# yigolden/JpegLibrary

Hardware: AMD Instinct MI355X
Metric: Mpixels/s decoded, 4K 4:2:0 baseline Q75 RST=4, 1 & 8 GPU vs CPU ref (higher is better)
Workload: dtype f32; 1 GPU; 1024 x 3840x2160 420 baseline Q75 DRI=4 per GPU, output interleaved_u8 resident in HBM; images_per_gpu=1024

## Files before the change

### jpeglibrary_amd/csrc/k3_idct.hip

```cpp
#include <hip/hip_runtime.h>
#include <stdint.h>

#include <algorithm>
#include <atomic>
#include <cstdio>
#include <cstdlib>

#include "common.h"
#include "kernels.h"
#include "encode_kernels.h"
#include "kernels_device.h"
#include "k3_index_math.h"

namespace jpgpu {


__device__ constexpr uint8_t kNat[64] = {0,  1,  8,  16, 9,  2,  3,  10, 17, 24, 32, 25, 18, 11, 4,  5,  12, 19, 26, 33, 40, 48,
                                         41, 34, 27, 20, 13, 6,  7,  14, 21, 28, 35, 42, 49, 56, 57, 50, 43, 36, 29, 22, 15, 23,
                                         30, 37, 44, 51, 58, 59, 52, 45, 38, 31, 39, 46, 53, 60, 61, 54, 47, 55, 62, 63};

static_assert(kIdctBlocksPerWg == 256, "the split form's reciprocals are exact for tiles of up to 256 blocks");
static_assert(kMaxBlocksPerMcu == 16, "kRecip16 and the 16-bit reciprocals of the split form cover 1..16 blocks per MCU");
__device__ constexpr uint32_t kRecip16[kMaxBlocksPerMcu + 1] = {0, 65536, 32768, 21846, 16384, 13108, 10923, 9363, 8192, 7282, 6554, 5958, 5462, 5042, 4682, 4370, 4096};

#define JPGPU_IDCT8(y0, y1, y2, y3, y4, y5, y6, y7)                     \
    {                                                                   \
        float mz0 = y1 + y7;                                            \
        float mz2 = y3 + y7;                                            \
        float mz1 = y3 + y5;                                            \
        float mz3 = y1 + y5;                                            \
        float mz4 = (mz0 + mz1) * 1.175875602f;                         \
        mz2 = (mz2 * -1.961570560f) + mz4;                              \
        mz3 = (mz3 * -0.390180644f) + mz4;                              \
        mz0 = mz0 * -0.899976223f;                                      \
        mz1 = mz1 * -2.562915447f;                                      \
        const float mb3 = ((y7 * 0.298631336f) + mz0) + mz2;            \
        const float mb2 = ((y5 * 2.053119869f) + mz1) + mz3;            \
        const float mb1 = ((y3 * 3.072711026f) + mz1) + mz2;            \
        const float mb0 = ((y1 * 1.501321110f) + mz0) + mz3;            \
        mz4 = (y2 + y6) * 0.541196100f;                                 \
        mz0 = y0 + y4;                                                  \
        mz1 = y0 - y4;                                                  \
        mz2 = mz4 + (y6 * -1.847759065f);                               \
        mz3 = mz4 + (y2 * 0.765366865f);                                \
        const float a0 = mz0 + mz3;                                     \
        const float a3 = mz0 - mz3;                                     \
        const float a1 = mz1 + mz2;                                     \
        const float a2 = mz1 - mz2;                                     \
        y0 = a0 + mb0;                                                  \
        y7 = a0 - mb0;                                                  \
        y1 = a1 + mb1;                                                  \
        y6 = a1 - mb1;                                                  \
        y2 = a2 + mb2;                                                  \
        y5 = a2 - mb2;                                                  \
        y3 = a3 + mb3;                                                  \
        y4 = a3 - mb3;                                                  \
    }

__device__ __forceinline__ void block_dequant(const uint8_t *c_lds, uint32_t swz, const uint16_t *q_lds, float (&f)[64]) {
#pragma unroll
    for (int piece = 0; piece < 8; piece++) {
        const uint4 cv = *reinterpret_cast<const uint4 *>(c_lds + ((piece ^ swz) * 16));
        const uint4 qv = reinterpret_cast<const uint4 *>(q_lds)[piece];
        const uint32_t cw[4] = {cv.x, cv.y, cv.z, cv.w};
        const uint32_t qw[4] = {qv.x, qv.y, qv.z, qv.w};
#pragma unroll
        for (int j = 0; j < 8; j++) {
            const int k = piece * 8 + j;
            const uint32_t w = cw[j >> 1], q = qw[j >> 1];
            const int32_t c = (j & 1) ? ((int32_t)w >> 16) : (int32_t)(int16_t)(w & 0xFFFF);
            const int32_t qq = (j & 1) ? (int32_t)(q >> 16) : (int32_t)(q & 0xFFFF);
            f[kNat[k]] = (float)(qq * c);
        }
    }
}

typedef float float2v __attribute__((ext_vector_type(2)));
typedef short short2v __attribute__((ext_vector_type(2)));
typedef unsigned short ushort2v __attribute__((ext_vector_type(2)));

template <typename T>
__device__ __forceinline__ void idct8(T &y0, T &y1, T &y2, T &y3, T &y4, T &y5, T &y6, T &y7) {
    T mz0 = y1 + y7;
    T mz2 = y3 + y7;
    T mz1 = y3 + y5;
    T mz3 = y1 + y5;
    T mz4 = (mz0 + mz1) * 1.175875602f;
    mz2 = (mz2 * -1.961570560f) + mz4;
    mz3 = (mz3 * -0.390180644f) + mz4;
    mz0 = mz0 * -0.899976223f;
    mz1 = mz1 * -2.562915447f;
    const T mb3 = ((y7 * 0.298631336f) + mz0) + mz2;
    const T mb2 = ((y5 * 2.053119869f) + mz1) + mz3;
    const T mb1 = ((y3 * 3.072711026f) + mz1) + mz2;
    const T mb0 = ((y1 * 1.501321110f) + mz0) + mz3;
    mz4 = (y2 + y6) * 0.541196100f;
    mz0 = y0 + y4;
    mz1 = y0 - y4;
    mz2 = mz4 + (y6 * -1.847759065f);
    mz3 = mz4 + (y2 * 0.765366865f);
    const T a0 = mz0 + mz3;
    const T a3 = mz0 - mz3;
    const T a1 = mz1 + mz2;
    const T a2 = mz1 - mz2;
    y0 = a0 + mb0;
    y7 = a0 - mb0;
    y1 = a1 + mb1;
    y6 = a1 - mb1;
    y2 = a2 + mb2;
    y5 = a2 - mb2;
    y3 = a3 + mb3;
    y4 = a3 - mb3;
}

__device__ __forceinline__ void block_idct(const float (&f)[64], int32_t level_shift, uint32_t (&out)[32]) {
#if defined(JPGPU_K3_PRICE)
#pragma unroll
    for (int i = 0; i < 32; i++) out[i] = (__builtin_bit_cast(uint32_t, f[2 * i]) >> 16) | (__builtin_bit_cast(uint32_t, f[2 * i + 1]) & 0xFFFF0000u) | (uint32_t)level_shift;
    return;
#endif
    float2v a[4][8];
#pragma unroll
    for (int r2 = 0; r2 < 4; r2++)
#pragma unroll
        for (int c = 0; c < 8; c++) a[r2][c] = float2v{f[(2 * r2) * 8 + c], f[(2 * r2 + 1) * 8 + c]};
#pragma unroll
    for (int r2 = 0; r2 < 4; r2++) idct8(a[r2][0], a[r2][1], a[r2][2], a[r2][3], a[r2][4], a[r2][5], a[r2][6], a[r2][7]);
    float2v b[8][4];
#pragma unroll
    for (int r2 = 0; r2 < 4; r2++)
#pragma unroll
        for (int c2 = 0; c2 < 4; c2++) {
            b[2 * r2][c2] = float2v{a[r2][2 * c2].x, a[r2][2 * c2 + 1].x};
            b[2 * r2 + 1][c2] = float2v{a[r2][2 * c2].y, a[r2][2 * c2 + 1].y};
        }
#pragma unroll
    for (int c2 = 0; c2 < 4; c2++) idct8(b[0][c2], b[1][c2], b[2][c2], b[3][c2], b[4][c2], b[5][c2], b[6][c2], b[7][c2]);
    const uint32_t shift2 = ((uint32_t)level_shift & 0xFFFFu) * 0x00010001u;
#pragma unroll
    for (int r = 0; r < 8; r++)
#pragma unroll
        for (int c2 = 0; c2 < 4; c2++) {
            const float2v v = b[r][c2] * 0.1250f;
            const int32_t x = (int32_t)__builtin_rintf(v.x);
            const int32_t y = (int32_t)__builtin_rintf(v.y);
            const uint32_t pk = ((uint32_t)x & 0xFFFFu) | ((uint32_t)y << 16);
            const short2v sum = __builtin_bit_cast(short2v, pk) + __builtin_bit_cast(short2v, shift2);
            out[r * 4 + c2] = __builtin_bit_cast(uint32_t, sum);
        }
}

__device__ __forceinline__ uint32_t clamp2_u8(uint32_t pk) {
    short2v v = __builtin_bit_cast(short2v, pk);
    v = __builtin_elementwise_max(v, short2v{0, 0});
    v = __builtin_elementwise_min(v, short2v{255, 255});
    return __builtin_bit_cast(uint32_t, v);
}
__device__ __forceinline__ uint32_t pack4_u8(uint32_t pk01, uint32_t pk23) {
    return __builtin_amdgcn_perm(clamp2_u8(pk23), clamp2_u8(pk01), 0x06040200u);
}
struct ScaleTo8 {
    uint32_t shift2, max2, mul2, rem2, mask2;
    bool expand;
};
__device__ __forceinline__ ScaleTo8 scale_to_8(uint32_t precision) {
    const uint32_t p = precision < 1u ? 1u : (precision > 16u ? 16u : precision);
    ScaleTo8 k;
    k.expand = p < 8u;
    const uint32_t pe = k.expand ? p : 1u;
    const uint32_t m = (uint32_t)(0x010101110955FFull >> (8u * (pe - 1u))) & 0xFFu;
    const uint32_t rem = 8u % pe;
    k.shift2 = (k.expand ? 0u : p - 8u) * 0x00010001u;
    k.max2 = ((1u << pe) - 1u) * 0x00010001u;
    k.mul2 = m * 0x00010001u;
    k.rem2 = rem * 0x00010001u;
    k.mask2 = ((1u << rem) - 1u) * 0x00010001u;
    return k;
}
__device__ __forceinline__ uint32_t shift_sat2_u8(uint32_t pk, const ScaleTo8 &k) {
    const uint32_t t = __builtin_bit_cast(uint32_t, __builtin_bit_cast(short2v, pk) >> __builtin_bit_cast(short2v, k.shift2));
    uint32_t r;
    asm("v_sat_pk_u8_i16 %0, %1" : "=v"(r) : "v"(t));
    return r;
}
__device__ __forceinline__ uint32_t expand2_u8(uint32_t pk, const ScaleTo8 &k) {
    short2v v = __builtin_bit_cast(short2v, pk);
    v = __builtin_elementwise_max(v, short2v{0, 0});
    v = __builtin_elementwise_min(v, __builtin_bit_cast(short2v, k.max2));
    const ushort2v r = __builtin_bit_cast(ushort2v, v) * __builtin_bit_cast(ushort2v, k.mul2);
    const ushort2v hi = r << __builtin_bit_cast(ushort2v, k.rem2);
    return __builtin_bit_cast(uint32_t, hi) | (__builtin_bit_cast(uint32_t, r) & k.mask2);
}
__device__ __forceinline__ uint32_t pick4(uint32_t lo, uint32_t hi, uint32_t sel) { return __builtin_amdgcn_perm(hi, lo, sel); }
#define JPGPU_SEL(a, b, c, d) ((uint32_t)(a) | ((uint32_t)(b) << 8) | ((uint32_t)(c) << 16) | ((uint32_t)(d) << 24))

constexpr int kIdctThreads = 256;
constexpr uint32_t kPxRowStride = kIdctThreads * 8;

enum IdctLayout : int { kLayGeneric = 0, kLayYccH1V1 = 1, kLayYccH2V1 = 2, kLayYccH2V2 = 3, kLayGray = 4, kNumIdctLayouts = 5 };

struct ChromaTerms {
    int32_t r, g, b;
};
__device__ __forceinline__ ChromaTerms chroma_terms(uint32_t cb_sample, uint32_t cr_sample, const YccRgbFactors &k) {
    const int32_t cb = (int32_t)cb_sample - 128, cr = (int32_t)cr_sample - 128;
    ChromaTerms t;
    t.r = (k.cr_r * cr + 32768) >> 16;
    t.b = (k.cb_b * cb + 32768) >> 16;
    t.g = (k.cb_g * cb + 32768 + k.cr_g * cr) >> 16;
    return t;
}
__device__ __forceinline__ uint32_t clamp_u8_i32(int32_t v) { return (uint32_t)(v < 0 ? 0 : (v > 255 ? 255 : v)); }
__device__ __forceinline__ uint32_t rgb_pixel(uint32_t y, const ChromaTerms &t) {
    return clamp_u8_i32((int32_t)y + t.r) | (clamp_u8_i32((int32_t)y + t.g) << 8) | (clamp_u8_i32((int32_t)y + t.b) << 16);
}
__device__ __forceinline__ uint32_t byte_of(uint32_t lo, uint32_t hi, int i) { return ((i < 4 ? lo : hi) >> (8 * (i & 3))) & 0xFFu; }
template <int N, int BPP>
__device__ __forceinline__ void store_rgb_pixels(uint8_t *dst, const uint32_t (&p)[N]) {
    if (BPP == 4) {
#pragma unroll
        for (int i = 0; i < N; i += 4) {
            const uint4 v = {p[i] | 0xFF000000u, p[i + 1] | 0xFF000000u, p[i + 2] | 0xFF000000u, p[i + 3] | 0xFF000000u};
            *reinterpret_cast<uint4 *>(dst + i * 4) = v;
        }
    } else {
        uint32_t w[N * 3 / 4];
#pragma unroll
        for (int i = 0; i < N; i += 4) {
            w[i * 3 / 4 + 0] = p[i] | (p[i + 1] << 24);
            w[i * 3 / 4 + 1] = (p[i + 1] >> 8) | (p[i + 2] << 16);
            w[i * 3 / 4 + 2] = (p[i + 2] >> 16) | (p[i + 3] << 8);
        }
        if (N == 16) {
#pragma unroll
            for (int i = 0; i < 3; i++) {
                const uint4 v = {w[i * 4], w[i * 4 + 1], w[i * 4 + 2], w[i * 4 + 3]};
                *reinterpret_cast<uint4 *>(dst + i * 16) = v;
            }
        } else {
#pragma unroll
            for (int i = 0; i < N * 3 / 8; i++) {
                const uint2 v = {w[i * 2], w[i * 2 + 1]};
                *reinterpret_cast<uint2 *>(dst + i * 8) = v;
            }
        }
    }
}

__global__ __launch_bounds__(256) void ycc_to_rgb_kernel(const uint8_t *__restrict__ src, uint8_t *__restrict__ dst, uint64_t n_pixels, int comps,
                                                         int bpp, YccRgbFactors k) {
    for (uint64_t i = (uint64_t)blockIdx.x * 256 + threadIdx.x; i < n_pixels; i += (uint64_t)gridDim.x * 256) {
        const uint32_t y = src[i * comps];
        const uint32_t cb = comps == 3 ? src[i * 3 + 1] : 128u, cr = comps == 3 ? src[i * 3 + 2] : 128u;
        const uint32_t px = rgb_pixel(y, chroma_terms(cb, cr, k));
        uint8_t *d = dst + i * bpp;
        d[0] = (uint8_t)px;
        d[1] = (uint8_t)(px >> 8);
        d[2] = (uint8_t)(px >> 16);
        if (bpp == 4) d[3] = 255;
    }
}

__global__ __launch_bounds__(256) void extend_u16_kernel(const uint8_t *__restrict__ planes, uint8_t *__restrict__ out_base,
                                                         const ExtendPlanes *__restrict__ images) {
    const ExtendPlanes g = images[blockIdx.y];
    uint16_t *out = reinterpret_cast<uint16_t *>(out_base + g.out_off);
    for (uint64_t px = (uint64_t)blockIdx.x * 256 + threadIdx.x; px < (uint64_t)g.width * g.height; px += (uint64_t)gridDim.x * 256) {
    const uint32_t y = (uint32_t)(px / g.width), x = (uint32_t)(px - (uint64_t)y * g.width);
    const uint32_t p = g.precision < 1u ? 1u : (g.precision > 16u ? 16u : g.precision), mx = (1u << p) - 1u;
    uint16_t v4[4] = {0, 0, 0, 0};
#pragma unroll
    for (uint32_t c = 0; c < 4u; c++) {
        if (c >= g.ncomp) continue;
        const int16_t *pl = reinterpret_cast<const int16_t *>(planes + g.plane_off[c]);
        const uint32_t mw = 8u * (g.max_h | (g.max_h == 0)), mh = 8u * (g.max_v | (g.max_v == 0));
        const uint32_t mcx = x / mw, pxm = x - mcx * mw, mcy = y / mh, pym = y - mcy * mh;
        const uint32_t bx = (pxm >> 3) < g.hcnt[c] - 1u ? (pxm >> 3) : g.hcnt[c] - 1u, by = (pym >> 3) < g.vcnt[c] - 1u ? (pym >> 3) : g.vcnt[c] - 1u;
        const uint32_t dx = pxm - 8u * bx, dy = pym - 8u * by;
        if (g.max_h != 0 && (dx >= (8u << g.hshift[c]) || dy >= (8u << g.vshift[c]))) continue;
        const uint32_t s = g.max_h == 0 ? (uint32_t)(uint16_t)pl[(uint64_t)(y >> g.vshift[c]) * g.pitch[c] + (x >> g.hshift[c])]
                                        : (uint32_t)(uint16_t)pl[(uint64_t)((mcy * g.vcnt[c] + by) * 8u + (dy >> g.vshift[c])) * g.pitch[c] + (mcx * g.hcnt[c] + bx) * 8u + (dx >> g.hshift[c])];
        uint32_t bits = s < mx ? s : mx;
        if (p >= 8u) {
            const uint32_t rem = 16u - p;
            bits = (bits << rem) | (bits & ((1u << rem) - 1u));
        } else {
            uint32_t cur = p;
            while (cur < 16u) {
                bits = (bits << p) | bits;
                cur += p;
            }
            if (cur > 16u) {
                bits >>= p;
                cur -= p;
                const uint32_t rem = 16u - cur;
                bits = (bits << rem) | (bits & ((1u << rem) - 1u));
            }
        }
        v4[c] = (uint16_t)bits;
    }
    *reinterpret_cast<uint2 *>(out + px * 4) = uint2{(uint32_t)v4[0] | ((uint32_t)v4[1] << 16), (uint32_t)v4[2] | ((uint32_t)v4[3] << 16)};
    }
}

template <int LAY, int CONV>
__device__ __forceinline__ void interleaved_output_from_tile(const uint8_t *sh_px, const DevScan &s, const K3TilePos &pos, uint32_t mpl,
                                                             uint32_t line_recip, uint32_t row_recip, uint32_t img_h, uint32_t n_mcu,
                                                             uint32_t tid, bool have_block, const DevScanComponent &comp, uint32_t mcu_x,
                                                             uint32_t mcu_y, uint32_t b, uint8_t *img, const YccRgbFactors &kf, bool reached,
                                                             uint32_t mcu, uint32_t fail_block) {
    if (LAY == kLayGeneric) {
        const uint32_t W = s.width, H = s.height, C = s.frame_components;
        if (have_block) {
            const uint32_t hs = comp.hs, vs = comp.vs;
            const bool flush = s.kind == kScanFrameOnly;
            const uint32_t x0 = flush ? (mcu_x * comp.h + s.blk_x[b]) * hs * 8 : (mcu_x * s.max_h + s.blk_x[b]) * 8;
            const uint32_t y0 = flush ? (mcu_y * comp.v + s.blk_y[b]) * vs * 8 : (mcu_y * s.max_v + s.blk_y[b]) * 8;
            const uint32_t hshift = 31 - __builtin_clz(hs | 1), vshift = 31 - __builtin_clz(vs | 1);
            const uint32_t bx = s.blk_x[b], by = s.blk_y[b];
            const bool overlap_h = !flush && comp.h > 1 && hs > 1, overlap_v = !flush && comp.v > 1 && vs > 1;
            const uint32_t base = b - (by * comp.h + bx);
            if ((overlap_h || overlap_v) && !reached) return;
            for (uint32_t v = 0; v < vs; v++)
                for (uint32_t i = 0; i < 8; i++) {
                    const uint32_t y = y0 + 8 * v + i;
                    if (y >= H) continue;
                    const uint8_t *srow = sh_px + ((8 * v + i) >> vshift) * kPxRowStride + tid * 8;
                    for (uint32_t h = 0; h < hs; h++) {
                        if (overlap_h || overlap_v) {
                            uint32_t later = 0xFFFFFFFFu;
                            if (overlap_h && bx + 1 < comp.h && h >= 1) later = base + by * comp.h + bx + 1;
                            else if (overlap_v && by + 1 < comp.v && v >= 1) {
                                const int32_t xf = (int32_t)bx + (int32_t)h - (int32_t)hs + 1;
                                later = base + (by + 1) * comp.h + (uint32_t)(xf < 0 ? 0 : xf);
                            }
                            if (later != 0xFFFFFFFFu && (uint64_t)mcu * s.blocks_per_mcu + later < fail_block) continue;
                        }
                        for (uint32_t j = 0; j < 8; j++) {
                            const uint32_t x = x0 + 8 * h + j;
                            if (x < W) img[((size_t)y * W + x) * C + comp.component_index] = srow[(8 * h + j) >> hshift];
                        }
                    }
                }
        }
    } else {
    constexpr uint32_t max_h = (LAY == kLayYccH1V1) ? 1 : 2;
    constexpr uint32_t max_v = (LAY == kLayYccH2V2) ? 2 : 1;
    constexpr uint32_t rows_per_mcu = 8 * max_v;
    constexpr uint32_t vshift = max_v >> 1;
    constexpr uint32_t kbpm = max_h * max_v + 2;
    constexpr uint32_t bpp = CONV == 4 ? 4 : 3;
    const uint32_t n_tasks = rows_per_mcu * n_mcu;
    const uint32_t W = mpl * (8 * max_h);
    const uint32_t y0 = pos.gy0 * rows_per_mcu;
    uint8_t *line0 = img + (uint64_t)y0 * W * bpp;
    for (uint32_t t = tid; t < n_tasks; t += kIdctThreads) {
        const uint32_t row = k3_task_row(t, row_recip), m = t - k3_mul24(row, n_mcu);
        const uint32_t x = pos.gx0 + m, wraps = k3_line_wraps(x, mpl, line_recip);
        uint32_t back = k3_mul24(wraps, mpl);
        asm("" : "+v"(back));
        const uint32_t gx = x - back;
        const uint32_t yl = wraps * rows_per_mcu + row;
        if (y0 + yl >= img_h) continue;
        const uint32_t mb = k3_mul24(m, kbpm);
        const uint8_t *yrow = sh_px + (row & 7) * kPxRowStride + (mb + (row >> 3) * max_h) * 8;
        const uint8_t *crow = sh_px + (row >> vshift) * kPxRowStride + (mb + max_h * max_v) * 8;
        uint8_t *dst_px = line0 + (k3_mul24(yl, W * bpp) + k3_mul24(gx, 8 * max_h * bpp));
        if (max_h == 2 && CONV != 0) {
            const uint4 yv = *reinterpret_cast<const uint4 *>(yrow);
            const uint4 cv = *reinterpret_cast<const uint4 *>(crow);
            uint32_t px[16];
#pragma unroll
            for (int j = 0; j < 8; j++) {
                const ChromaTerms t = chroma_terms(byte_of(cv.x, cv.y, j), byte_of(cv.z, cv.w, j), kf);
                px[2 * j] = rgb_pixel(byte_of(j < 4 ? yv.x : yv.z, j < 4 ? yv.y : yv.w, (2 * j) & 7), t);
                px[2 * j + 1] = rgb_pixel(byte_of(j < 4 ? yv.x : yv.z, j < 4 ? yv.y : yv.w, (2 * j + 1) & 7), t);
            }
            store_rgb_pixels<16, bpp>(dst_px, px);
        } else if (CONV != 0) {
            const uint2 yv = *reinterpret_cast<const uint2 *>(yrow);
            const uint2 bv = *reinterpret_cast<const uint2 *>(crow);
            const uint2 rv = *reinterpret_cast<const uint2 *>(crow + 8);
            uint32_t px[8];
#pragma unroll
            for (int j = 0; j < 8; j++) px[j] = rgb_pixel(byte_of(yv.x, yv.y, j), chroma_terms(byte_of(bv.x, bv.y, j), byte_of(rv.x, rv.y, j), kf));
            store_rgb_pixels<8, bpp>(dst_px, px);
        } else if (max_h == 2) {
            const uint4 yv = *reinterpret_cast<const uint4 *>(yrow);
            const uint4 cv = *reinterpret_cast<const uint4 *>(crow);
            const uint32_t cc0 = pick4(cv.x, cv.z, JPGPU_SEL(0, 4, 1, 5)), cc1 = pick4(cv.x, cv.z, JPGPU_SEL(2, 6, 3, 7));
            const uint32_t cc2 = pick4(cv.y, cv.w, JPGPU_SEL(0, 4, 1, 5)), cc3 = pick4(cv.y, cv.w, JPGPU_SEL(2, 6, 3, 7));
            uint4 o0, o1, o2;
            o0.x = pick4(yv.x, cc0, JPGPU_SEL(0, 4, 5, 1));
            o0.y = pick4(yv.x, cc0, JPGPU_SEL(4, 5, 2, 6));
            o0.z = pick4(yv.x, cc0, JPGPU_SEL(7, 3, 6, 7));
            o0.w = pick4(yv.y, cc1, JPGPU_SEL(0, 4, 5, 1));
            o1.x = pick4(yv.y, cc1, JPGPU_SEL(4, 5, 2, 6));
            o1.y = pick4(yv.y, cc1, JPGPU_SEL(7, 3, 6, 7));
            o1.z = pick4(yv.z, cc2, JPGPU_SEL(0, 4, 5, 1));
            o1.w = pick4(yv.z, cc2, JPGPU_SEL(4, 5, 2, 6));
            o2.x = pick4(yv.z, cc2, JPGPU_SEL(7, 3, 6, 7));
            o2.y = pick4(yv.w, cc3, JPGPU_SEL(0, 4, 5, 1));
            o2.z = pick4(yv.w, cc3, JPGPU_SEL(4, 5, 2, 6));
            o2.w = pick4(yv.w, cc3, JPGPU_SEL(7, 3, 6, 7));
            uint4 *dst = reinterpret_cast<uint4 *>(dst_px);
            dst[0] = o0;
            dst[1] = o1;
            dst[2] = o2;
        } else {
            const uint2 yv = *reinterpret_cast<const uint2 *>(yrow);
            const uint2 bv = *reinterpret_cast<const uint2 *>(crow);
            const uint2 rv = *reinterpret_cast<const uint2 *>(crow + 8);
            uint2 o0, o1, o2;
            {
                const uint32_t lo = pick4(bv.x, rv.x, JPGPU_SEL(0, 4, 1, 5)), hi = pick4(bv.x, rv.x, JPGPU_SEL(2, 6, 3, 7));
                const uint32_t mid = pick4(lo, hi, JPGPU_SEL(2, 3, 4, 5));
                o0.x = pick4(yv.x, lo, JPGPU_SEL(0, 4, 5, 1));
                o0.y = pick4(yv.x, mid, JPGPU_SEL(4, 5, 2, 6));
                o1.x = pick4(yv.x, hi, JPGPU_SEL(5, 3, 6, 7));
            }
            {
                const uint32_t lo = pick4(bv.y, rv.y, JPGPU_SEL(0, 4, 1, 5)), hi = pick4(bv.y, rv.y, JPGPU_SEL(2, 6, 3, 7));
                const uint32_t mid = pick4(lo, hi, JPGPU_SEL(2, 3, 4, 5));
                o1.y = pick4(yv.y, lo, JPGPU_SEL(0, 4, 5, 1));
                o2.x = pick4(yv.y, mid, JPGPU_SEL(4, 5, 2, 6));
                o2.y = pick4(yv.y, hi, JPGPU_SEL(5, 3, 6, 7));
            }
            uint2 *dst = reinterpret_cast<uint2 *>(dst_px);
            dst[0] = o0;
            dst[1] = o1;
            dst[2] = o2;
        }
    }
    }
}

typedef __attribute__((address_space(3))) void jpgpu_lds_void;
typedef const __attribute__((address_space(1))) void jpgpu_gbl_void;

template <int FMT, int LAY, bool PRE, bool SPLIT = false>
__device__ __forceinline__ void idct_output_body(
    const int16_t *__restrict__ coefs, const DevScan *__restrict__ scans, const IdctWork *__restrict__ work,
    const DevScanStatus *__restrict__ status, const DevQuantTable *__restrict__ quant_pool, uint8_t *__restrict__ out, YccRgbFactors kf) {
    constexpr int CONV = FMT == kFmtRgbU8 ? 3 : (FMT == kFmtRgbaU8 ? 4 : 0);
    constexpr bool kSampleBytes = fmt_is_sample_bytes(FMT);
    __shared__ __attribute__((aligned(16))) uint8_t sh_all[kIdctThreads * 128 + kIdctThreads * 64 + kMaxScanComponents * 128 + (SPLIT && !PRE ? 64 : 0)];
    uint8_t *sh = sh_all;
    uint8_t *sh_px = sh_all + kIdctThreads * 128;
    uint16_t(*sh_q)[64] = reinterpret_cast<uint16_t(*)[64]>(sh_all + kIdctThreads * 128 + kIdctThreads * 64);
    uint8_t *sh_flag = sh_all + kIdctThreads * 128 + kIdctThreads * 64 + kMaxScanComponents * 128;

    const IdctWork wk = work[blockIdx.x];
    const DevScan &s = scans[wk.scan];
    const uint32_t tid = threadIdx.x;
    const uint32_t wave = tid >> 6;
    const uint32_t bpm = s.blocks_per_mcu;
    const uint32_t mcus_per_tile = wk.mcus_per_tile;
    uint32_t decoded = status ? status[wk.scan].decoded_mcus : s.total_mcus;
    if (decoded > s.total_mcus) decoded = s.total_mcus;
    uint32_t fail_block = 0xFFFFFFFFu;
    if (status != nullptr && s.kind == kScanSequential) {
        const uint32_t fb = status[wk.scan].pad[1];
        if (fb != 0) fail_block = kFailBlockBase - fb;
        for (uint32_t j = s.first_scan; j < wk.scan; j++)
            if (scans[j].image_index == s.image_index && status[j].first_error != kNoError) fail_block = 0;
    }
    const bool keep = (s.shadow_mask & kKeepUnreachedMcus) != 0;
    constexpr bool kPerMcuLayout = fmt_is_interleaved(FMT) && (LAY == kLayYccH1V1 || LAY == kLayYccH2V1 || LAY == kLayYccH2V2);
    uint32_t first_mcu = wk.first_mcu;
    uint32_t range_end = wk.first_mcu + wk.n_mcus;
    if (first_mcu == kIdctPartialMcu) {
        if (fail_block == 0xFFFFFFFFu || fail_block % bpm == 0 || fail_block / bpm >= decoded) return;
        first_mcu = fail_block / bpm;
        range_end = first_mcu + 1;
    } else if (keep) {
        const uint32_t reach = kPerMcuLayout ? fail_block / bpm : (fail_block == 0xFFFFFFFFu ? fail_block : (fail_block + bpm - 1) / bpm);
        if (range_end > decoded) range_end = decoded;
        if (range_end > reach) range_end = reach;
        if (first_mcu >= range_end) return;
    }

    if (tid < (uint32_t)s.scan_components * 32) {
        const uint32_t c = tid >> 5, i = tid & 31;
        reinterpret_cast<uint32_t *>(sh_q[c])[i] =
            reinterpret_cast<const uint32_t *>(quant_pool[s.quant_pool[s.comp[c].quant_slot]].q)[i];
    }

    const uint32_t mcu_local = tid / bpm;
    const uint32_t b = tid - mcu_local * bpm;
    const uint32_t ci_early = s.blk_comp[b < kMaxBlocksPerMcu ? b : 0];
    const uint8_t *coef_bytes = reinterpret_cast<const uint8_t *>(coefs + s.coef_off * 64);

    auto tile_mcus = [&](uint32_t first) { return (range_end - first) < mcus_per_tile ? (range_end - first) : mcus_per_tile; };
    const uint32_t tile_blocks = mcus_per_tile * bpm;
    constexpr bool split = SPLIT && !PRE;
    if (split && (s.reserved0 & kScanSplitHandoff) == 0) return;
    const uint32_t sp_dri = split ? s.dri : 1u;
    const uint32_t sp_rb = kRecip16[bpm <= (uint32_t)kMaxBlocksPerMcu ? bpm : 0];
    const uint32_t sp_rd = __builtin_amdgcn_readfirstlane(sp_dri <= 256u ? ((1u << 20) + sp_dri - 1) / sp_dri : 0u);
    const uint32_t sp_w = sp_dri * bpm;
    const bool sp_fast = split && mcus_per_tile % (2 * sp_dri) == 0 && first_mcu % (2 * sp_dri) == 0;
    const uint32_t sp_rw = __builtin_amdgcn_readfirstlane((65536u + sp_w - 1) / sp_w);
    const uint8_t *sp_hi = coef_bytes + split_plane_lines(s.n_intervals, sp_dri, bpm) * 128;
    const uint8_t *sp_flags = reinterpret_cast<const uint8_t *>(reinterpret_cast<const uint64_t *>(coefs) + (s.reserved0 >> kSplitFlagShift));
    auto sp_locate = [&](uint32_t tile_first, uint32_t t, uint32_t k, uint32_t &line, uint32_t &iv, uint32_t &word) {
        const uint32_t i0 = __builtin_amdgcn_readfirstlane(tile_first / sp_dri), m0 = tile_first - i0 * sp_dri;
        const uint32_t blk = k * 32 + (t >> 3);
        uint32_t q = (blk * sp_rb) >> 16;
        const uint32_t bb = blk - q * bpm;
        const uint32_t last = s.total_mcus - 1 - tile_first;
        q = q < last ? q : last;
        const uint32_t mm = m0 + q;
        const uint32_t by_mul = (mm * sp_rd) >> 20, by_cmp = mm >= sp_dri ? 1u : 0u;
        const uint32_t qi = sp_dri > 256u ? by_cmp : by_mul;
        const uint32_t m = mm - qi * sp_dri;
        iv = i0 + qi;
        line = ((iv >> 1) * sp_dri + m) * bpm + bb;
        word = ((iv >> 6) * sp_dri + m) * bpm + bb;
    };
    auto sp_locate_fast = [&](uint32_t i0, uint32_t t, uint32_t k, uint32_t &iv, uint32_t &word) {
        const uint32_t ll = k * 16 + ((t >> 3) & 15u);
        const uint32_t pp = (ll * sp_rw) >> 16;
        iv = i0 + 2 * pp + ((t >> 7) & 1u);
        iv = iv < s.n_intervals ? iv : s.n_intervals - 1;
        word = (iv >> 6) * sp_w + (ll - pp * sp_w);
    };
    auto sp_own_block = [&](uint32_t t) {
        const uint32_t ml = (t * sp_rb) >> 16, bb = t - ml * bpm;
        const uint32_t ir = (ml * sp_rd) >> 20, m = ml - ir * sp_dri;
        const uint32_t ll = ((ir >> 1) * sp_dri + m) * bpm + bb;
        return ((ll >> 4) << 5) | ((ir & 1u) << 4) | (ll & 15u);
    };
    const uint32_t sp_ipt = __builtin_amdgcn_readfirstlane(mcus_per_tile / sp_dri);
    uint32_t sp_i0 = __builtin_amdgcn_readfirstlane(first_mcu / sp_dri);
    auto sp_load_flag = [&](uint32_t tile_first, uint32_t tile_i0, uint32_t &fb, uint32_t &bit_at) {
        uint32_t t_ = tid;
        asm volatile("" : "+v"(t_));
        const uint32_t k = t_ >> 5, t8 = (t_ & 31u) << 3;
        uint32_t line, iv, word;
        if (sp_fast) sp_locate_fast(tile_i0, t8, k, iv, word);
        else sp_locate(tile_first, t8, k, line, iv, word);
        fb = sp_flags[word * 8 + ((iv >> 3) & 7u)];
        bit_at = iv & 7u;
    };
    auto sp_wait_seen = [&]() {
        if (split) __builtin_amdgcn_s_waitcnt(0x0070);
    };
    auto sp_publish_flags = [&](uint32_t fb, uint32_t bit_at, uint32_t set) {
        asm volatile("" : "+v"(fb));
        const uint64_t w = __builtin_amdgcn_ballot_w64(((fb >> bit_at) & 1u) != 0);
        if ((tid & 63u) == 0) *reinterpret_cast<uint2 *>(sh_flag + set * 32 + wave * 8) = uint2{(uint32_t)w, (uint32_t)(w >> 32)};
    };
    auto sp_read_flags = [&](uint32_t set) {
        const uint4 lo = *reinterpret_cast<const uint4 *>(sh_flag + set * 32), hi = *reinterpret_cast<const uint4 *>(sh_flag + set * 32 + 16);
        const uint32_t w[8] = {lo.x, lo.y, lo.z, lo.w, hi.x, hi.y, hi.z, hi.w};
        const uint32_t at = tid >> 3;
        uint32_t bits = 0;
#pragma unroll
        for (int k = 0; k < 8; k++) bits |= ((w[k] >> at) & 1u) << k;
        return bits;
    };
    auto dma_tile = [&](uint32_t tile_first, uint32_t tile_i0, uint32_t hi_bits) {
        uint32_t t_ = tid;
        asm volatile("" : "+v"(t_));
        if (split && sp_fast) {
            const uint32_t piece = (t_ & 7) ^ ((t_ >> 4) & 7);
            const uint32_t slot = ((t_ >> 3) & 15u) * 2 + (t_ >> 7);
            const uint8_t *src = (piece < 4 ? coef_bytes : sp_hi) + (uint64_t)(tile_i0 >> 1) * sp_w * 128 + (slot * 64 + (piece & 3u) * 16);
            const uint8_t *zeros = sp_flags - 128 + (piece & 3u) * 16;
            const uint32_t fetch_bits = piece < 4 ? 0xFFu : hi_bits;
#pragma unroll
            for (int k = 0; k < 8; k++) {
                const uint8_t *from = ((fetch_bits >> k) & 1u) ? src + (uint32_t)(k * 2048) : zeros;
                if (k < 6 || (uint32_t)k * 32 + slot < tile_blocks)
                    __builtin_amdgcn_global_load_lds((jpgpu_gbl_void *)from, (jpgpu_lds_void *)(sh + ((uint32_t)k * kIdctThreads + wave * 64) * 16), 16, 0, 0);
            }
            return;
        }
        if (split) {
            const uint32_t piece = (t_ & 7) ^ ((t_ >> 4) & 7);
#pragma unroll
            for (int k = 0; k < 8; k++) {
                uint32_t line, iv, word;
                sp_locate(tile_first, t_, k, line, iv, word);
                const bool wanted = k < 6 || (uint32_t)k * 32 + (t_ >> 3) < tile_blocks;
                const bool fetch = wanted && (piece < 4 || ((hi_bits >> k) & 1u) != 0);
                const uint8_t *src = (piece < 4 ? coef_bytes : sp_hi) + ((uint64_t)line * 128 + (iv & 1u) * 64 + (piece & 3u) * 16);
                if (fetch)
                    __builtin_amdgcn_global_load_lds((jpgpu_gbl_void *)src, (jpgpu_lds_void *)(sh + ((uint32_t)k * kIdctThreads + wave * 64) * 16), 16, 0, 0);
                if (wanted && !fetch) *reinterpret_cast<uint4 *>(sh + ((uint32_t)k * kIdctThreads + t_) * 16) = uint4{0, 0, 0, 0};
            }
            return;
        }
        const uint32_t dma_lane_off = (t_ >> 3) * 128 + (((t_ & 7) ^ ((t_ >> 4) & 7)) * 16);
        const uint8_t *src = coef_bytes + (uint64_t)tile_first * bpm * 128;
#pragma unroll
        for (int k = 0; k < 8; k++)
            if (k < 6 || (uint32_t)k * 32 + (tid >> 3) < tile_blocks)
                __builtin_amdgcn_global_load_lds((jpgpu_gbl_void *)(src + (uint32_t)(k * 4096) + dma_lane_off),
                                                 (jpgpu_lds_void *)(sh + ((uint32_t)k * kIdctThreads + wave * 64) * 16), 16, 0, 0);
    };

    uint32_t hi_next = 0;
    if (split) {
        const uint32_t n_sets = first_mcu + mcus_per_tile < range_end ? 2u : 1u;
#pragma nounroll
        for (uint32_t set = 0; set < n_sets; set++) {
            uint32_t fb, at;
            sp_load_flag(first_mcu + set * mcus_per_tile, sp_i0 + set * sp_ipt, fb, at);
            asm volatile("s_waitcnt vmcnt(0)" ::: "memory");
            sp_wait_seen();
            sp_publish_flags(fb, at, set);
        }
        __syncthreads();
        const uint32_t hi_first = sp_read_flags(0);
        if (n_sets == 2) hi_next = sp_read_flags(1);
        dma_tile(first_mcu, sp_i0, hi_first);
    } else {
        dma_tile(first_mcu, sp_i0, 0);
    }
    const uint32_t mpl = __builtin_amdgcn_readfirstlane(s.mcus_per_line);
    const uint32_t line_recip = __builtin_amdgcn_readfirstlane(k3_line_recip(mpl));
    const uint32_t img_h = __builtin_amdgcn_readfirstlane((uint32_t)s.height);
    uint8_t *const img = out + s.out_off;
    K3TilePos pos = k3_tile_pos(first_mcu, mpl);
    pos.gx0 = __builtin_amdgcn_readfirstlane(pos.gx0);
    pos.gy0 = __builtin_amdgcn_readfirstlane(pos.gy0);
    K3TilePos pos_step = k3_tile_pos(mcus_per_tile, mpl);
    pos_step.gx0 = __builtin_amdgcn_readfirstlane(pos_step.gx0);
    pos_step.gy0 = __builtin_amdgcn_readfirstlane(pos_step.gy0);
    const uint32_t row_recip_full = __builtin_amdgcn_readfirstlane(k3_row_recip(mcus_per_tile));
    const uint32_t row_recip_last = __builtin_amdgcn_readfirstlane(k3_row_recip((range_end - first_mcu - 1) % mcus_per_tile + 1));
    asm volatile("s_waitcnt vmcnt(0)" ::: "memory");
    __syncthreads();

  for (uint32_t tile_first = first_mcu; tile_first < range_end; tile_first += mcus_per_tile) {
    const uint32_t n_mcu = tile_mcus(tile_first);
    const uint32_t n_blk = n_mcu * bpm;
    const uint32_t next_first = tile_first + mcus_per_tile;
    const bool have_next = next_first < range_end;

    const uint32_t mcu = tile_first + mcu_local;
    const bool have_block = tid < n_blk;
    bool writes = have_block && ((s.shadow_mask >> ci_early) & 1u) == 0;

    float f[64];
    uint32_t px[32];
    if (PRE) {
        if (have_block) {
#pragma unroll
            for (int piece = 0; piece < 8; piece++) {
                const uint4 cv = *reinterpret_cast<const uint4 *>(sh + tid * 128 + ((piece ^ ((tid >> 1) & 7)) * 16));
                px[piece * 4] = cv.x;
                px[piece * 4 + 1] = cv.y;
                px[piece * 4 + 2] = cv.z;
                px[piece * 4 + 3] = cv.w;
            }
        }
    } else {
        constexpr bool kPerTile = split || (FMT == kFmtRgbU8 && (LAY == kLayYccH2V1 || LAY == kLayYccH2V2)) || (kSampleBytes && LAY == kLayGeneric);
        uint32_t t_ = tid;
        if (kPerTile) asm volatile("" : "+v"(t_));
        if (split && sp_fast) t_ = sp_own_block(t_);
        if (have_block) block_dequant(sh + t_ * 128, (t_ >> 1) & 7, sh_q[ci_early], f);
    }
    asm volatile("s_waitcnt lgkmcnt(0)" ::: "memory");
    __builtin_amdgcn_s_barrier();
    if (have_next) dma_tile(next_first, sp_i0 + sp_ipt, hi_next);
    hi_next = 0;

    if (!PRE && have_block) block_idct(f, (int32_t)s.level_shift, px);
    uint32_t sp_fb = 0, sp_at = 0;
    const bool sp_ahead = split && next_first + mcus_per_tile < range_end;
    if (sp_ahead) sp_load_flag(next_first + mcus_per_tile, sp_i0 + 2 * sp_ipt, sp_fb, sp_at);
    sp_i0 += sp_ipt;
    const bool reached = mcu < decoded && mcu * bpm + b < fail_block;
    if ((s.shadow_mask & 0xFu) == 0) {
        writes = writes && (reached || !keep);
    } else {
        const uint32_t bb = b < kMaxBlocksPerMcu ? b : 0u, me = s.blk_comp[bb], fc = s.comp[me & 3u].component_index;
        uint32_t later = 0xFFu, earlier = 0xFFu;
        for (uint32_t cc = 0; cc < s.scan_components && cc < (uint32_t)kMaxScanComponents; cc++) {
            if (cc == me || s.comp[cc].component_index != fc) continue;
            if (cc > me && later == 0xFFu) later = cc;
            if (cc < me) earlier = cc;
        }
        uint32_t first_me = 0xFFu, first_later = 0xFFu, first_earlier = 0xFFu;
        for (uint32_t k = 0; k < bpm && k < (uint32_t)kMaxBlocksPerMcu; k++) {
            const uint32_t ck = s.blk_comp[k];
            if (ck == me && first_me == 0xFFu) first_me = k;
            if (ck == later && first_later == 0xFFu) first_later = k;
            if (ck == earlier && first_earlier == 0xFFu) first_earlier = k;
        }
        const bool later_reached = later != 0xFFu && mcu < decoded && mcu * bpm + (b - first_me + first_later) < fail_block;
        const bool earlier_reached = earlier != 0xFFu && mcu < decoded && mcu * bpm + (b - first_me + first_earlier) < fail_block;
        writes = have_block && (reached ? !later_reached : (!keep && later == 0xFFu && !earlier_reached));
    }
    if (!reached) {
#pragma unroll
        for (int i = 0; i < 32; i++) px[i] = 0;
    }
    bool synced = false;
    uint32_t ml_late = mcu_local, b_late = b;
    asm volatile("" : "+v"(ml_late), "+v"(b_late));
    const uint32_t mcu_wraps = k3_line_wraps(pos.gx0 + ml_late, mpl, line_recip);
    uint32_t mcu_back = k3_mul24(mcu_wraps, mpl);
    asm("" : "+v"(mcu_back));
    const uint32_t mcu_y = pos.gy0 + mcu_wraps, mcu_x = pos.gx0 + ml_late - mcu_back;
    const uint32_t ci = s.blk_comp[b_late < kMaxBlocksPerMcu ? b_late : 0];
    const DevScanComponent comp = s.comp[ci];
    const uint32_t b_out = split ? b_late : b;
// ... 286 lines not shown
```

Measured before the change: 629,900 Mpixels/s.

## Exchange output pieces across lane quads via DPP so stores coalesce contiguously

```diff
diff --git a/jpeglibrary_amd/csrc/k3_idct.hip b/jpeglibrary_amd/csrc/k3_idct.hip
--- a/jpeglibrary_amd/csrc/k3_idct.hip
+++ b/jpeglibrary_amd/csrc/k3_idct.hip
@@ -11,6 +11,7 @@
 #include "encode_kernels.h"
 #include "kernels_device.h"
 #include "k3_index_math.h"
+#include "k3_store_quads.h"
 
 namespace jpgpu {
 
@@ -302,6 +303,43 @@
     *reinterpret_cast<uint2 *>(out + px * 4) = uint2{(uint32_t)v4[0] | ((uint32_t)v4[1] << 16), (uint32_t)v4[2] | ((uint32_t)v4[3] << 16)};
     }
 }
+
+struct QuadKeepMasks {
+    uint64_t ne0, ne1, ne2, ne3;
+};
+__device__ __forceinline__ QuadKeepMasks quad_keep_masks(bool exchange) {
+    return QuadKeepMasks{exchange ? 0xEEEEEEEEEEEEEEEEull : ~0ull, exchange ? 0xDDDDDDDDDDDDDDDDull : ~0ull, exchange ? 0xBBBBBBBBBBBBBBBBull : ~0ull,
+                         exchange ? 0x7777777777777777ull : ~0ull};
+}
+constexpr bool quad_move_is(uint32_t store, uint32_t lane, uint32_t src_lane, uint32_t src_reg) {
+    return k3_quad_move(store, lane).src_lane == src_lane && k3_quad_move(store, lane).src_reg == src_reg;
+}
+static_assert(quad_move_is(0, 0, 0, 0) && quad_move_is(0, 1, 1, 0) && quad_move_is(0, 2, 0, 1) && quad_move_is(0, 3, 0, 2), "store 0 of the assembly below");
+static_assert(quad_move_is(1, 0, 1, 2) && quad_move_is(1, 1, 1, 1) && quad_move_is(1, 2, 2, 1) && quad_move_is(1, 3, 2, 0), "store 1 of the assembly below");
+static_assert(quad_move_is(2, 0, 3, 0) && quad_move_is(2, 1, 3, 1) && quad_move_is(2, 2, 2, 2) && quad_move_is(2, 3, 3, 2), "store 2 of the assembly below");
+#define JPGPU_QSEL(d, from, keep, src) \
+    "v_cndmask_b32_dpp " d ", " from ", " keep ", vcc quad_perm:[" src "," src "," src "," src "] row_mask:0xf bank_mask:0xf bound_ctrl:1\n\t"
+#define JPGPU_QSEL4(d, from, keep, src) \
+    JPGPU_QSEL("%[" d "x]", "%[" from "x]", "%[" keep "x]", src) JPGPU_QSEL("%[" d "y]", "%[" from "y]", "%[" keep "y]", src) \
+    JPGPU_QSEL("%[" d "z]", "%[" from "z]", "%[" keep "z]", src) JPGPU_QSEL("%[" d "w]", "%[" from "w]", "%[" keep "w]", src)
+__device__ __forceinline__ void quad_exchange(const uint4 &o0, const uint4 &o1, const uint4 &o2, const QuadKeepMasks &k, uint4 &d0, uint4 &d1, uint4 &d2) {
+    asm volatile("s_nop 4\n\t"
+        "s_mov_b64 vcc, %[ne2]\n\t"
+        JPGPU_QSEL4("d0", "o1", "o0", "0")
+        "s_mov_b64 vcc, %[ne0]\n\t"
+        JPGPU_QSEL4("d1", "o2", "o1", "1") JPGPU_QSEL4("d2", "o0", "o2", "3")
+        "s_mov_b64 vcc, %[ne3]\n\t"
+        JPGPU_QSEL4("d0", "o2", "d0", "0") JPGPU_QSEL4("d1", "o0", "d1", "2")
+        "s_mov_b64 vcc, %[ne1]\n\t"
+        JPGPU_QSEL4("d2", "o1", "d2", "3")
+        : [d0x] "=&v"(d0.x), [d0y] "=&v"(d0.y), [d0z] "=&v"(d0.z), [d0w] "=&v"(d0.w), [d1x] "=&v"(d1.x), [d1y] "=&v"(d1.y), [d1z] "=&v"(d1.z),
+          [d1w] "=&v"(d1.w), [d2x] "=&v"(d2.x), [d2y] "=&v"(d2.y), [d2z] "=&v"(d2.z), [d2w] "=&v"(d2.w)
+        : [o0x] "v"(o0.x), [o0y] "v"(o0.y), [o0z] "v"(o0.z), [o0w] "v"(o0.w), [o1x] "v"(o1.x), [o1y] "v"(o1.y), [o1z] "v"(o1.z), [o1w] "v"(o1.w),
+          [o2x] "v"(o2.x), [o2y] "v"(o2.y), [o2z] "v"(o2.z), [o2w] "v"(o2.w), [ne0] "s"(k.ne0), [ne1] "s"(k.ne1), [ne2] "s"(k.ne2), [ne3] "s"(k.ne3)
+        : "vcc");
+}
+#undef JPGPU_QSEL4
+#undef JPGPU_QSEL
 
 template <int LAY, int CONV>
 __device__ __forceinline__ void interleaved_output_from_tile(const uint8_t *sh_px, const DevScan &s, const K3TilePos &pos, uint32_t mpl,
@@ -354,6 +392,12 @@
     const uint32_t W = mpl * (8 * max_h);
     const uint32_t y0 = pos.gy0 * rows_per_mcu;
     uint8_t *line0 = img + (uint64_t)y0 * W * bpp;
+    constexpr bool kQuads = CONV == 0 && max_h == 2;
+    const bool exchange = kQuads && k3_quad_eligible(n_mcu, mpl, pos.gx0);
+    const QuadKeepMasks keep = quad_keep_masks(exchange);
+    uint32_t q_off[kK3QuadStores];
+#pragma unroll
+    for (uint32_t st = 0; st < kK3QuadStores; st++) q_off[st] = exchange ? k3_quad_lane_offset(k3_quad_offsets_packed(st), tid) : st * kK3QuadPieceBytes;
     for (uint32_t t = tid; t < n_tasks; t += kIdctThreads) {
         const uint32_t row = k3_task_row(t, row_recip), m = t - k3_mul24(row, n_mcu);
         const uint32_t x = pos.gx0 + m, wraps = k3_line_wraps(x, mpl, line_recip);
@@ -365,7 +409,8 @@
         const uint32_t mb = k3_mul24(m, kbpm);
         const uint8_t *yrow = sh_px + (row & 7) * kPxRowStride + (mb + (row >> 3) * max_h) * 8;
         const uint8_t *crow = sh_px + (row >> vshift) * kPxRowStride + (mb + max_h * max_v) * 8;
-        uint8_t *dst_px = line0 + (k3_mul24(yl, W * bpp) + k3_mul24(gx, 8 * max_h * bpp));
+        const uint32_t at = k3_mul24(yl, W * bpp) + k3_mul24(gx, 8 * max_h * bpp);
+        uint8_t *dst_px = line0 + at;
         if (max_h == 2 && CONV != 0) {
             const uint4 yv = *reinterpret_cast<const uint4 *>(yrow);
             const uint4 cv = *reinterpret_cast<const uint4 *>(crow);
@@ -403,10 +448,18 @@
             o2.y = pick4(yv.w, cc3, JPGPU_SEL(0, 4, 5, 1));
             o2.z = pick4(yv.w, cc3, JPGPU_SEL(4, 5, 2, 6));
             o2.w = pick4(yv.w, cc3, JPGPU_SEL(7, 3, 6, 7));
-            uint4 *dst = reinterpret_cast<uint4 *>(dst_px);
-            dst[0] = o0;
-            dst[1] = o1;
-            dst[2] = o2;
+            if (kQuads) {
+                uint4 d0, d1, d2;
+                quad_exchange(o0, o1, o2, keep, d0, d1, d2);
+                *reinterpret_cast<uint4 *>(line0 + (at + q_off[0])) = d0;
+                *reinterpret_cast<uint4 *>(line0 + (at + q_off[1])) = d1;
+                *reinterpret_cast<uint4 *>(line0 + (at + q_off[2])) = d2;
+            } else {
+                uint4 *dst = reinterpret_cast<uint4 *>(dst_px);
+                dst[0] = o0;
+                dst[1] = o1;
+                dst[2] = o2;
+            }
         } else {
             const uint2 yv = *reinterpret_cast<const uint2 *>(yrow);
             const uint2 bv = *reinterpret_cast<const uint2 *>(crow);
diff --git a/jpeglibrary_amd/csrc/k3_store_quads.h b/jpeglibrary_amd/csrc/k3_store_quads.h
--- /dev/null
+++ b/jpeglibrary_amd/csrc/k3_store_quads.h
@@ -0,0 +1,42 @@
+#pragma once
+#include <stdint.h>
+
+#ifndef JPGPU_HD
+#if defined(__HIPCC__) || defined(__CUDACC__)
+#define JPGPU_HD __host__ __device__
+#else
+#define JPGPU_HD
+#endif
+#endif
+
+namespace jpgpu {
+
+constexpr uint32_t kK3QuadStores = 3, kK3QuadLanes = 4, kK3QuadPieceBytes = 16;
+
+struct K3QuadMove {
+    uint8_t src_lane, src_reg, piece;
+};
+JPGPU_HD constexpr K3QuadMove k3_quad_move(uint32_t store, uint32_t lane) {
+    constexpr K3QuadMove table[kK3QuadStores][kK3QuadLanes] = {
+        {{0, 0, 0}, {1, 0, 3}, {0, 1, 1}, {0, 2, 2}},
+        {{1, 2, 5}, {1, 1, 4}, {2, 1, 7}, {2, 0, 6}},
+        {{3, 0, 9}, {3, 1, 10}, {2, 2, 8}, {3, 2, 11}},
+    };
+    return table[store][lane];
+}
+
+JPGPU_HD constexpr uint32_t k3_quad_offsets_packed(uint32_t store) {
+    uint32_t packed = 0;
+    for (uint32_t lane = 0; lane < kK3QuadLanes; lane++) {
+        const int32_t sixteenths = (int32_t)k3_quad_move(store, lane).piece - 3 * (int32_t)lane;
+        packed |= ((uint32_t)sixteenths & 0xFFu) << (8 * lane);
+    }
+    return packed;
+}
+JPGPU_HD inline uint32_t k3_quad_lane_offset(uint32_t packed, uint32_t lane) {
+    return (uint32_t)((int32_t)(int8_t)(packed >> (8 * (lane & 3u))) * (int32_t)kK3QuadPieceBytes);
+}
+
+JPGPU_HD inline bool k3_quad_eligible(uint32_t n_mcu, uint32_t mpl, uint32_t gx0) { return ((n_mcu | mpl | gx0) & 3u) == 0; }
+
+}
```

New measurement: 644,900 Mpixels/s, median of 6. 1.02x the previous value.
